# LikeLy-Journey/SegmenTron

Hardware: AMD Instinct MI355X
Metric: images/sec fwd+bwd DeepLabv3+_xception65 @1025x2049 (higher is better)
Workload: dtype bf16; 1 GPU; DeepLabv3+_xception65 train step (fwd + CE loss + bwd + SGD) @1025x2049, batch 2/GPU (BASELINE.json configs[2]); global_batch=2, bn=BN, parallelism=dp1, full_size=True

## Files before the change

### include/segmentron_hip.h

```cpp
#ifndef SEGMENTRON_HIP_H
#define SEGMENTRON_HIP_H
#ifdef __cplusplus
extern "C" {
#endif

const char* seg_last_error(void);
int seg_version(void);

int seg_fast_div_host(const int* s, long n, int d, int* q);
int seg_fast_div_exact(long s, long d);
int seg_fast_div_max_quot(long* out);

int seg_conv_gemm_fwd(int dtype, const void* x, long ldx, int N, int Hi, int Wi, int C,
                      const void* w, int O, int KH, int KW, int stride, int pad, int dil,
                      int pro_mode, const float* pro_scale, const float* pro_shift,
                      const float* bias, void* y, long ldy, int Ho, int Wo, int out_H, int out_W,
                      int out_s, float* stat_partial, const void* ep_x, long ldep,
                      const float* ep_c0, const float* ep_c1, int tconv, void* stream);
int seg_conv_gemm_tiles_m(int N, int Ho, int Wo);

int seg_conv_gemm_wgrad(int dtype, const void* x, long ldx, int N, int Hi, int Wi, int C,
                        const void* dy, long lddy, int Ho, int Wo, int O, int KH, int KW,
                        int stride, int pad, int dil, int pro_mode, const float* pro_scale,
                        const float* pro_shift, float* partial, int splits, void* stream);
int seg_conv_gemm_stat_rows(int dtype, int N, int Ho, int Wo, int C, int O, int KH, int KW,
                            int stride, int pad, int dil, int tconv, int has_bias, int pro_mode);
int seg_conv_gemm_wgrad_splits(int dtype, int N, int Ho, int Wo, int C, int O, int KH, int KW,
                               int stride, int pad, int dil, int pro_mode);

int seg_dwconv3x3(int dtype, int mode, const void* x, long ldx, int N, int Hi, int Wi, int C,
                  const float* w9c, int w_layout, int stride, int dil, int pro_mode,
                  const float* pro_scale, const float* pro_shift, void* y, long ldy, int Ho, int Wo,
                  float* stat_partial, int grid_y, void* stream);
int seg_dwconv_grid_y(int dtype, int C, int N, int Ho, int Wo, int stride, int dil, int kind);
int seg_dwconv3x3_wgrad_finalize(const float* partial, int R, int C, float* dw_c9, void* stream);
int seg_dwconv3x3_wgrad(int dtype, const void* x, long ldx, int N, int Hi, int Wi, int C,
                        const void* dy, long lddy, int Ho, int Wo, int stride, int dil,
                        int pro_mode, const float* pro_scale, const float* pro_shift,
                        float* partial, int grid_y, void* stream);

int seg_dwconv3x3_bwd_fused(int dtype, const void* dy, long lddy, const void* x, long ldx, int N,
                            int H, int W, int C, const float* w9c, int w_layout, int dil,
                            int pro_mode, const float* pro_scale, const float* pro_shift, void* g,
                            long ldg, float* partial_w, float* partial_bn, int grid_y,
                            void* stream);
int seg_dwconv3x3_bwd_fused_add_ok(int dil);
int seg_dwconv3x3_bwd_fused_add(int dtype, const void* dy, long lddy, const void* x, long ldx, int N,
                                int H, int W, int C, const float* w9c, int w_layout, int pro_mode,
                                const float* pro_scale, const float* pro_shift, const void* res,
                                long ldr, void* g, long ldg, float* partial_w, float* partial_bn,
                                int grid_y, void* stream);
int seg_dwconv3x3_bwd_fused_sum_ok(int dtype, int C, int dil);
int seg_dwconv3x3_bwd_fused_sum(int dtype, const void* dy, long lddy, const void* x, long ldx, int N,
                                int H, int W, int C, const float* w9c, int w_layout, int pro_mode,
                                const float* pro_scale, const float* pro_shift, const void* res,
                                long ldr, void* g, long ldg, float* partial_w, float* partial_bn,
                                int grid_y, void* stream);

int seg_colsum(const float* in, long R, int L, double* out_d, float* out_f, double* ws,
               void* stream);
int seg_colsum_count(const float* in, long R, int L, double* out_d, double count, double* ws,
                     void* stream);
int seg_bn_finalize(const double* sums, double count, const double* count_dev,
                    const float* gamma, const float* beta, float eps, float momentum, float* running_mean, float* running_var,
                    float* mean, float* invstd, float* scale, float* shift, int C,
                    const float* mean_offset, void* stream);
int seg_bn_finalize_p(const float* partial, long R, double count, const float* gamma,
                      const float* beta, float eps, float momentum, float* running_mean,
                      float* running_var, float* mean, float* invstd, float* scale, float* shift,
                      int C, const float* mean_offset, double* ws, void* stream);
int seg_bn_finalize_small(int dtype, const void* y, long ldy, long M, int C, const float* gamma,
                          const float* beta, float eps, float momentum, float* running_mean,
                          float* running_var, float* mean, float* invstd, float* scale,
                          float* shift, const float* mean_offset, void* stream);
int seg_bn_moments_small(int dtype, const void* y, long ldy, long M, int C, double* moments,
                         void* stream);
int seg_bn_finalize_small_sync(void* p2p, int dtype, const void* y, long ldy, long M, int C,
                               const float* gamma, const float* beta, float eps, float momentum,
                               float* running_mean, float* running_var, float* mean, float* invstd,
                               float* scale, float* shift, const float* mean_offset,
                               double* count_out, void* stream);
int seg_sum_n(int dtype, int n, const void* const* xs, const long* lds, void* y, long ldy, long M,
              int C, void* stream);
int seg_bn_eval_affine(const float* gamma, const float* beta, const float* rm, const float* rv,
                       float eps, float* scale, float* shift, int C, void* stream);
int seg_bn_eval_affine_multi(int n, const float* const* gamma, const float* const* beta,
                             const float* const* rm, const float* const* rv, const float* eps,
                             float* const* out, const int* C, void* stream);
int seg_bn_apply(int dtype, const void* x, long ldx, int mode_x, const float* sx, const float* tx,
                 const void* r, long ldr, int mode_r, const float* sr, const float* tr,
// ... 219 lines not shown
```

### segmentron_amd/csrc/dwconv_slide.hip

```cpp
#include <type_traits>
#include "common.h"
#include "dwconv.h"

namespace seg {

constexpr int SL_THREADS = 256, SL_CQ = 16, SL_WL = 16;
constexpr int SL_DEPTH_F = 2, SL_OCC_F = 4, SL_DEPTH_B = 2;
#define SL_SCHED_BARRIER() __builtin_amdgcn_sched_barrier(0)

struct DwSlideArgs {
  const void* x;
  const void* dy;
  const void* res;
  void* y;
  const float* w;
  int w_layout;
  const float* sc; const float* sh;
  float* partial;
  float* partial_bn;
  long ldx, lddy, ldy, ldr;
  int N, H, W, C, pro_mode, rs, nstrips, nwblk, ncblk;
};

struct SlBlock { int n, strip, wblk, cblk, prow; };
__device__ __forceinline__ SlBlock sl_block(const DwSlideArgs& a) {
  const int nblk = a.ncblk * a.nwblk * a.nstrips * a.N;
  int L = xcd_remap(blockIdx.x, nblk);
  SlBlock b;
  b.cblk = L % a.ncblk;
  L /= a.ncblk;
  b.prow = L;
  b.wblk = L % a.nwblk;
  L /= a.nwblk;
  b.strip = L % a.nstrips;
  b.n = L / a.nstrips;
  return b;
}

typedef float f32x2 __attribute__((ext_vector_type(2)));
typedef short s16x2 __attribute__((ext_vector_type(2)));
struct Q4 { f32x2 lo, hi; };
__device__ __forceinline__ Q4 q4_zero() { Q4 q; q.lo = q.hi = (f32x2){0.f, 0.f}; return q; }
__device__ __forceinline__ void q4_fma(Q4& acc, const Q4& a, const Q4& b) {
  acc.lo = __builtin_elementwise_fma(a.lo, b.lo, acc.lo);
  acc.hi = __builtin_elementwise_fma(a.hi, b.hi, acc.hi);
}
template <typename T> struct SlIO;
template <> struct SlIO<bf16_t> {
  typedef uint2 raw_t;
  static constexpr int BYTES = 8;
  __device__ static __forceinline__ Q4 unpack(const raw_t& r) {
    Q4 q;
    q.lo = (f32x2){__uint_as_float(r.x << 16), __uint_as_float(r.x & 0xFFFF0000u)};
    q.hi = (f32x2){__uint_as_float(r.y << 16), __uint_as_float(r.y & 0xFFFF0000u)};
// ... 60 lines not shown
      const float4 v = *reinterpret_cast<const float4*>(a.w + (long)tap * a.C + c);
      wt[k].lo = (f32x2){v.x, v.y};
      wt[k].hi = (f32x2){v.z, v.w};
    }
  }
}

template <int MODE, bool RELU_DONE>
__device__ __forceinline__ void sl_act(Q4& q, const Q4& sc, const Q4& sh) {
  const f32x2 z = {0.f, 0.f}, six = {6.f, 6.f};
  if (MODE & PRO_AFFINE) {
    q.lo = __builtin_elementwise_fma(q.lo, sc.lo, sh.lo);
    q.hi = __builtin_elementwise_fma(q.hi, sc.hi, sh.hi);
  }
  if ((MODE & PRO_RELU) && !RELU_DONE) {
    q.lo = __builtin_elementwise_max(q.lo, z);
    q.hi = __builtin_elementwise_max(q.hi, z);
  }
  if (MODE & PRO_CLAMP6) {
    q.lo = __builtin_elementwise_min(q.lo, six);
    q.hi = __builtin_elementwise_min(q.hi, six);
  }
}

struct SlThread {
  int c, w, r0, r1, rlast;
  bool live, lm, rm;
  unsigned off_m, off_0, off_p;
  bool edge, first, last;
  unsigned off_e;
  int bp_up, bp_dn;
};
template <int ESIZE>
__device__ __forceinline__ SlThread sl_thread(const DwSlideArgs& a, const SlBlock& b, long ld) {
  const int tid = threadIdx.x, cq = tid & (SL_CQ - 1), wl = tid >> 4;
  SlThread t;
  const int cfull = (b.cblk * SL_CQ + cq) * 4, wfull = b.wblk * SL_WL + wl;
  t.c = min(cfull, a.C - 4);
  t.w = min(wfull, a.W - 1);
  t.live = wfull < a.W && cfull < a.C;
  t.lm = t.w >= 1;
  t.rm = t.w + 1 < a.W;
  t.r0 = b.strip * a.rs;
  t.r1 = min(a.H, t.r0 + a.rs);
  t.rlast = min(t.r1, a.H - 1);
  t.off_m = (unsigned)((max(t.w - 1, 0) * ld + t.c) * ESIZE);
  t.off_0 = (unsigned)((t.w * ld + t.c) * ESIZE);
  t.off_p = (unsigned)((min(t.w + 1, a.W - 1) * ld + t.c) * ESIZE);
  const int lane = tid & 63, col = lane >> 4;
  t.first = col == 0;
  t.last = col == 3;
  t.edge = t.first || t.last;
  t.off_e = t.first ? t.off_m : (t.last ? t.off_p : 0xFFFFFFFFu);
  t.bp_up = ((lane - 16) & 63) * 4;
  t.bp_dn = ((lane + 16) & 63) * 4;
  return t;
}

typedef unsigned int sl_u32x2 __attribute__((ext_vector_type(2)));
typedef unsigned int sl_u32x4 __attribute__((ext_vector_type(4)));
template <typename R> __device__ __forceinline__ R sl_ld_edge(const unsigned char* row, unsigned nbytes, unsigned off);
template <> __device__ __forceinline__ uint2 sl_ld_edge<uint2>(const unsigned char* row, unsigned nbytes, unsigned off) {
  const __amdgpu_buffer_rsrc_t r = __builtin_amdgcn_make_buffer_rsrc((void*)row, 0, (int)nbytes, 0x00020000);
  const sl_u32x2 v = __builtin_amdgcn_raw_buffer_load_b64(r, (int)off, 0, 0);
  return make_uint2(v.x, v.y);
}
template <> __device__ __forceinline__ uint4 sl_ld_edge<uint4>(const unsigned char* row, unsigned nbytes, unsigned off) {
  const __amdgpu_buffer_rsrc_t r = __builtin_amdgcn_make_buffer_rsrc((void*)row, 0, (int)nbytes, 0x00020000);
  const sl_u32x4 v = __builtin_amdgcn_raw_buffer_load_b128(r, (int)off, 0, 0);
  return make_uint4(v.x, v.y, v.z, v.w);
}
template <typename R> __device__ __forceinline__ void sl_st_row(unsigned char* row, unsigned nbytes, unsigned off, const R& v);
template <> __device__ __forceinline__ void sl_st_row<uint2>(unsigned char* row, unsigned nbytes, unsigned off, const uint2& v) {
  const __amdgpu_buffer_rsrc_t r = __builtin_amdgcn_make_buffer_rsrc((void*)row, 0, (int)nbytes, 0x00020000);
  const sl_u32x2 d = {v.x, v.y};
  __builtin_amdgcn_raw_buffer_store_b64(d, r, (int)off, 0, 0);
}
template <> __device__ __forceinline__ void sl_st_row<uint4>(unsigned char* row, unsigned nbytes, unsigned off, const uint4& v) {
  const __amdgpu_buffer_rsrc_t r = __builtin_amdgcn_make_buffer_rsrc((void*)row, 0, (int)nbytes, 0x00020000);
  const sl_u32x4 d = {v.x, v.y, v.z, v.w};
  __builtin_amdgcn_raw_buffer_store_b128(d, r, (int)off, 0, 0);
// ... 296 lines not shown
#pragma unroll
  for (int k = 0; k < 9; ++k) {
    const int kw = k % 3;
    const bool keep = t.live && (kw != 2 || t.lm) && (kw != 0 || t.rm);
    v[k * 4] = keep ? accw[k].lo.x : 0.f; v[k * 4 + 1] = keep ? accw[k].lo.y : 0.f;
    v[k * 4 + 2] = keep ? accw[k].hi.x : 0.f; v[k * 4 + 3] = keep ? accw[k].hi.y : 0.f;
  }
  v[36] = s1.lo.x; v[37] = s1.lo.y; v[38] = s1.hi.x; v[39] = s1.hi.y;
  v[40] = s2.lo.x; v[41] = s2.lo.y; v[42] = s2.hi.x; v[43] = s2.hi.y;
#pragma unroll
  for (int i = 36; i < 44; ++i) v[i] = t.live ? v[i] : 0.f;
#pragma unroll
  for (int i = 0; i < 44; ++i) {
    v[i] += __shfl_xor(v[i], 16, 64);
    v[i] += __shfl_xor(v[i], 32, 64);
  }
  __shared__ float red[4][SL_CQ][44];
  if ((tid & 63) < SL_CQ) {
#pragma unroll
    for (int i = 0; i < 44; ++i) red[tid >> 6][cq][i] = v[i];
  }
  __syncthreads();
  for (int e = tid; e < SL_CQ * 44; e += SL_THREADS) {
    const int q = e / 44, k = e - q * 44;
    const float tot = red[0][q][k] + red[1][q][k] + red[2][q][k] + red[3][q][k];
    const int ch = (b.cblk * SL_CQ + q) * 4 + (k & 3), r = k >> 2;
    if (ch < a.C) {
      if (r < 9) a.partial[((long)b.prow * 9 + r) * a.C + ch] = tot;
      else if (a.partial_bn != nullptr) a.partial_bn[((long)b.prow * 2 + (r - 9)) * a.C + ch] = tot;
    }
  }
}

static void slide_geom(DwSlideArgs& a, int N, int H, int W, int C) {
  a.ncblk = (C / 4 + SL_CQ - 1) / SL_CQ;
  a.nwblk = (W + SL_WL - 1) / SL_WL;
  long ns = (H + 21) / 43;
  const long per_strip = (long)N * a.nwblk * a.ncblk;
  const long want = (400 + per_strip - 1) / per_strip;
  if (ns < want) ns = want;
  if (ns > H / 8) ns = H / 8;
  const long cap = 1024 / ((long)N * a.nwblk);
  if (ns > cap) ns = cap;
  if (ns < 1) ns = 1;
  a.rs = (int)((H + ns - 1) / ns);
  a.nstrips = (H + a.rs - 1) / a.rs;
}

int dw_slide_rows(int C, int N, int H, int W) {
  DwSlideArgs a;
  slide_geom(a, N, H, W, C);
  return N * a.nstrips * a.nwblk;
}

static bool slide_exchange(const DwSlideArgs& a, int esize) {
  return (long)a.N * a.H * a.W * a.C * esize >= (30L << 20);
}
template <typename T>
static void slide_launch_fwd(const DwSlideArgs& a, dim3 grid, hipStream_t st) {
  const bool xc = slide_exchange(a, (int)sizeof(T));
  switch (a.pro_mode) {
#define SL_CASE(M)                                                                                  \
  case M:                                                                                           \
    if (xc) hipLaunchKernelGGL((dwconv_slide_fwd_kernel<T, M, true>), grid, dim3(SL_THREADS), 0, st, a);  \
    else hipLaunchKernelGGL((dwconv_slide_fwd_kernel<T, M, false>), grid, dim3(SL_THREADS), 0, st, a);    \
    break;
    SL_CASE(0) SL_CASE(1) SL_CASE(2) SL_CASE(3) SL_CASE(5) SL_CASE(7)
#undef SL_CASE
    default: break;
  }
}
template <typename T, int RES>
static void slide_launch_bwd(const DwSlideArgs& a, dim3 grid, hipStream_t st) {
  const bool xc = slide_exchange(a, (int)sizeof(T));
  switch (a.pro_mode) {
#define SL_CASE(M)                                                                                       \
  case M:                                                                                                \
    if (xc) hipLaunchKernelGGL((dwconv_slide_bwd_kernel<T, M, RES, true>), grid, dim3(SL_THREADS), 0, st, a);  \
    else hipLaunchKernelGGL((dwconv_slide_bwd_kernel<T, M, RES, false>), grid, dim3(SL_THREADS), 0, st, a);    \
    break;
    SL_CASE(0) SL_CASE(1) SL_CASE(2) SL_CASE(3) SL_CASE(5) SL_CASE(7)
#undef SL_CASE
    default: break;
  }
}
static bool slide_mode_ok(int m) { return m == 0 || m == 1 || m == 2 || m == 3 || m == 5 || m == 7; }

int launch_dw_slide_fwd(int dtype, const void* x, long ldx, int N, int H, int W, int C,
                        const float* w, int w_layout, int pro_mode, const float* sc,
                        const float* sh, void* y, long ldy, float* stat_partial, int rows,
                        hipStream_t st) {
  DwSlideArgs a;
  a.x = x; a.dy = nullptr; a.res = nullptr; a.y = y; a.w = w; a.w_layout = w_layout;
  a.sc = sc; a.sh = sh; a.partial = stat_partial; a.partial_bn = nullptr;
  a.ldx = ldx; a.lddy = 0; a.ldy = ldy; a.ldr = 0;
  a.N = N; a.H = H; a.W = W; a.C = C; a.pro_mode = pro_mode;
  slide_geom(a, N, H, W, C);
  SEG_REQUIRE(slide_mode_ok(pro_mode), "dwconv (slide): unsupported prologue mode %d", pro_mode);
  SEG_REQUIRE(C % 4 == 0 && ldx % 4 == 0 && ldy % 4 == 0,
              "dwconv (slide): C/ldx/ldy must be multiples of 4");
  SEG_REQUIRE(stat_partial == nullptr || rows == N * a.nstrips * a.nwblk,
              "dwconv (slide): %d partial rows, the launch writes %d (seg_dwconv_grid_y)", rows,
              N * a.nstrips * a.nwblk);
  const dim3 grid((unsigned)((long)a.ncblk * a.nwblk * a.nstrips * N));
  if (dtype == DT_BF16) slide_launch_fwd<bf16_t>(a, grid, st);
  else slide_launch_fwd<float>(a, grid, st);
  return check_launch("dwconv3x3 (slide)");
}

int launch_dw_slide_bwd(int dtype, const void* dy, long lddy, const void* x, long ldx, int N, int H,
                        int W, int C, const float* w, int w_layout, int pro_mode, const float* sc,
                        const float* sh, void* g, long ldg, float* partial_w, float* partial_bn,
                        int rows, hipStream_t st, const void* res, long ldr, int res_mode) {
  DwSlideArgs a;
  a.x = x; a.dy = dy; a.res = res; a.y = g; a.w = w; a.w_layout = w_layout & 1;
  a.sc = sc; a.sh = sh; a.partial = partial_w; a.partial_bn = partial_bn;
  a.ldx = ldx; a.lddy = lddy; a.ldy = ldg; a.ldr = ldr;
  a.N = N; a.H = H; a.W = W; a.C = C; a.pro_mode = pro_mode;
  slide_geom(a, N, H, W, C);
  SEG_REQUIRE(slide_mode_ok(pro_mode), "dwconv bwd (slide): unsupported prologue mode %d", pro_mode);
  SEG_REQUIRE(C % 4 == 0 && ldx % 4 == 0 && lddy % 4 == 0 && ldg % 4 == 0 &&
                  (res == nullptr || ldr % 4 == 0),
              "dwconv bwd (slide): C/ldx/lddy/ldg/ldr must be multiples of 4");
  SEG_REQUIRE(rows == N * a.nstrips * a.nwblk,
              "dwconv bwd (slide): %d partial rows, the launch writes %d (seg_dwconv_grid_y)", rows,
              N * a.nstrips * a.nwblk);
  const dim3 grid((unsigned)((long)a.ncblk * a.nwblk * a.nstrips * N));
  const int rm = !res ? SL_RES_NONE : res_mode;
  SEG_REQUIRE(rm >= SL_RES_NONE && rm <= SL_RES_SUM, "dwconv bwd (slide): residual mode %d", rm);
  if (dtype == DT_BF16) {
    if (rm == SL_RES_SUM) slide_launch_bwd<bf16_t, SL_RES_SUM>(a, grid, st);
    else if (rm == SL_RES_POST) slide_launch_bwd<bf16_t, SL_RES_POST>(a, grid, st);
    else slide_launch_bwd<bf16_t, SL_RES_NONE>(a, grid, st);
  } else {
    if (rm == SL_RES_SUM) slide_launch_bwd<float, SL_RES_SUM>(a, grid, st);
    else if (rm == SL_RES_POST) slide_launch_bwd<float, SL_RES_POST>(a, grid, st);
    else slide_launch_bwd<float, SL_RES_NONE>(a, grid, st);
  }
  return check_launch("dwconv3x3_bwd_fused (slide)");
}

}
```

### segmentron_amd/functional.py

```python
import contextlib
import dataclasses
import os
import weakref

import torch
import torch.distributed as dist
import torch.nn as nn

from . import hip_ops as K
from . import parallel
from .hip_ops import PRO_AFFINE, PRO_NONE, PRO_RELU


class BNState:
    __slots__ = ("gamma", "beta", "mean", "invstd", "scale", "shift", "count", "training", "group")

    def __init__(self, gamma, beta, mean, invstd, scale, shift, count, training, group=None):
        self.gamma, self.beta = gamma, beta
        self.mean, self.invstd, self.scale, self.shift = mean, invstd, scale, shift
        self.count, self.training, self.group = count, training, group


RELU, RELU6 = 1, 5

# ... 336 lines not shown
    if KH == 1 and KW == 1 and opad == O:
        out = torch.empty((Cw, O), dtype=dtype, device=w.device)
        out.copy_(w.detach().reshape(O, Cw).t())
        return out
    p = w.detach().flip(2, 3).permute(1, 2, 3, 0)
    if opad != O:
        p = torch.nn.functional.pad(p, (0, opad - O))
    return p.reshape(Cw, KH * KW * opad).to(dtype).contiguous()


def pack_conv_weight_tconv(w, opad, dtype):
    O, Cw, KH, KW = w.shape
    p = w.detach().permute(1, 2, 3, 0)
    if opad != O:
        p = torch.nn.functional.pad(p, (0, opad - O))
    return p.reshape(Cw, KH * KW * opad).to(dtype).contiguous()


def pack_dw_weight(w, flipped=False):
    C = w.shape[0]
    t = w.detach().reshape(C, 9)
    if flipped:
        t = t.flip(1)
    out = torch.empty((9, C), dtype=torch.float32, device=w.device)
    out.copy_(t.t())
    return out


def _dw_taps(weight, stride, dil, reversed=False):
    if K.dw_tiled(stride, dil):
        return weight.detach()
    return cached_pack(weight, "dw_flip" if reversed else "dw",
                       lambda: pack_dw_weight(weight, reversed))


def _dw_bwd_is_fused(stride, dil, C, wdtype):
    return stride == 1 or (stride == 2 and dil == 1 and C % 4 == 0 and wdtype == torch.float32)


def _round_up(v, m):
    return (v + m - 1) // m * m


class ConvSpec:

    def __init__(self, act, stride=1, pad=0, dil=1, out=None, want_stats=True):
        self.bn_in, self.relu = act.bn, act.relu
        self.pro = act.pro
        self.stride, self.pad, self.dil = stride, pad, dil
        self.out, self.want_stats = out, want_stats
        self.partial = None
        self.drop_bias = False
        self.fork = None
        self.park = None


class _ConvFn(torch.autograd.Function):

    @staticmethod
    def forward(ctx, x, in_gamma, in_beta, weight, bias, spec):
        O, Cw, KH, KW = weight.shape
        cx, dt = x.shape[-1], x.dtype
        if KH == 1 and KW == 1 and cx == Cw and weight.dtype == torch.float32:
            wp = packed_pointwise(weight, False, dt)
        else:
            wp = cached_pack(weight, ("fwd", cx, dt), lambda: pack_conv_weight(weight, cx, dt))
# ... 125 lines not shown
        if box is not None and isinstance(bn.count, torch.Tensor):
            dgamma, dbeta, c0, c1 = K.fold_bwd_finalize_sync(
                box, dsdt, bn.count, bn.mean, bn.invstd, bn.gamma, bn.scale,
                parallel.grad_scale(bn.group))
        else:
            if bn.group is not None:
                dsdt = K.colsum(dsdt, f64=False)
                parallel.allreduce_backward_sums(dsdt, bn.group)
            dgamma, dbeta, c0, c1 = K.fold_bwd_finalize(
                dsdt, bn.count, bn.mean, bn.invstd, bn.gamma, bn.scale,
                parallel.grad_scale(bn.group) if bn.group is not None else 1.0)
        dx = None
        if ctx.needs_input_grad[0]:
            if s.stride == 1:
                dx, _ = K.conv_gemm(dy, ctx.wpt, C, 1, 1, 1, 0, 1,
                                    ep=(x, c0, c1) if bn.training else None)
            else:
                g, _ = K.conv_gemm(dy, ctx.wpt, C, 1, 1, 1, 0, 1,
                                   scatter=(x.shape[1], x.shape[2], s.stride))
                if bn.training:
                    ones = _ones(C, x.device)
                    dx = K.bn_bwd_apply(g, x, (PRO_AFFINE, ones, ones), c0, c1, out=g)
                else:
                    dx = g
            if s.park is not None and s.park.can_park(GradFork.RAW, dx, x):
                s.park.g, dx = dx, None
        return dx, dgamma, dbeta, dW.view_as(weight), None


class _DwFn(torch.autograd.Function):

    @staticmethod
    def forward(ctx, x, in_gamma, in_beta, weight, spec):
        y, spec.partial = K.dwconv(x, _dw_taps(weight, spec.stride, spec.dil), spec.stride,
                                   spec.dil, spec.pro, spec.out, spec.want_stats)
        spec.out = None
        ctx.spec = spec
        ctx.save_for_backward(x, weight)
        return y

    @staticmethod
    def backward(ctx, dy):
        x, weight = ctx.saved_tensors
        s = ctx.spec
        C = weight.shape[0]
        if K.nhwc(dy)[4] % K.vec_of(dy.dtype) != 0:
            dy = dy.contiguous()
        dx = dgamma = dbeta = None
        bn = s.bn_in
        f = s.fork
        if f is not None:
            f.closed = True
        tiled = K.dw_tiled(s.stride, s.dil)
        fused = _dw_bwd_is_fused(s.stride, s.dil, C, weight.dtype)
        fused_s2 = fused and s.stride == 2
        if ctx.needs_input_grad[0] and fused:
            raw = bn is not None and (fused_s2 or tiled) and \
                (bn.group is None or (parallel.mailbox(bn.group) is not None
                                      and isinstance(bn.count, torch.Tensor)))
            if fused_s2:
                g, dW, pb = K.dwconv_bwd_fused_s2(x, dy, weight.detach().contiguous(), s.pro,
                                                  want_bn=bn is not None, raw_dw=raw)
            else:
                res, as_sum = None, False
                if f is not None and f.g is not None and f.kind in (GradFork.POST, GradFork.SUM):
                    as_sum = f.kind == GradFork.SUM
                    if bn is None and (K.dwconv_bwd_fused_sum_ok(x.dtype, C, s.dil) if as_sum
                                       else K.dwconv_bwd_fused_add_ok(s.dil)):
                        res = s.fork.take()
                        if res.dtype != x.dtype or tuple(res.shape) != tuple(x.shape):
                            s.fork.g, res = res, None
                g, dW, pb = K.dwconv_bwd_fused(x, dy, _dw_taps(weight, 1, s.dil), s.dil, s.pro,
                                               want_bn=bn is not None, torch_layout=tiled,
                                               raw_dw=raw, res=res, res_sum=as_sum)
                if not tiled:
                    dW = K.dw_torch_layout(dW)
            if bn is None:
                dx = g
            else:
                dgamma, dbeta, c0, c1, dWsum = _bn_bwd_finish(pb, bn, dW if raw else None)
                if raw:
                    dW = dWsum
                if not bn.training:
                    c0 = c1 = None
                add = add_pro = None
                if f is not None and f.g is not None and f.kind in (GradFork.RAW, GradFork.PRE) \
                        and f.g.dtype == g.dtype and tuple(f.g.shape) == tuple(g.shape):
                    add_pro = f.coef if f.kind == GradFork.PRE else None
                    add = f.take()
                dx = K.bn_bwd_apply(g, x, (PRO_AFFINE, bn.scale, bn.shift), c0, c1, out=g, add=add,
                                    add_pro=add_pro)
        else:
            dW = K.dwconv_wgrad(x, dy, s.stride, s.dil, s.pro, torch_layout=tiled)
            if not tiled:
                dW = K.dw_torch_layout(dW)
            if ctx.needs_input_grad[0]:
                w = _dw_taps(weight, s.stride, s.dil, reversed=s.stride == 1)
                g = K.dwconv_dgrad(dy, w, s.stride, s.dil, (x.shape[1], x.shape[2]))
                dx, dgamma, dbeta = bn_input_backward(g, x, bn, s.relu, inplace=True)
        if f is not None and f.g is not None and dx is not None:
            if f.kind == GradFork.PRE:
                raise RuntimeError("a gradient parked for the depthwise backward's BatchNorm pass "
                                   "was not taken (stride %d, dilation %d, C %d)"
                                   % (s.stride, s.dil, C))
            dx = dx + f.take()
        return dx, dgamma, dbeta, dW, None

# ... 881 lines not shown
```

### segmentron_amd/hip_ops.py

```python
import torch

from ._lib import LIB

PRO_NONE, PRO_RELU, PRO_AFFINE, PRO_AFFINE_RELU = 0, 1, 2, 3
_DT = {torch.float32: 0, torch.bfloat16: 1}


def vec_of(dtype):
    return 8 if dtype == torch.bfloat16 else 4


_raw_stream = getattr(torch._C, "_cuda_getCurrentRawStream", None)


def _stream():
    if _raw_stream is not None:
        return _raw_stream(torch.cuda.current_device())
    return torch.cuda.current_stream().cuda_stream


def _p(t):
    return 0 if t is None else t.data_ptr()


# ... 249 lines not shown
def dwconv_bwd_fused_add_ok(dil):
    return bool(LIB.query("seg_dwconv3x3_bwd_fused_add_ok", int(dil)))


def dwconv_bwd_fused_sum_ok(dtype, C, dil):
    return bool(LIB.query("seg_dwconv3x3_bwd_fused_sum_ok", _DT[dtype], int(C), int(dil)))


def dwconv_bwd_fused(x, dy, w, dil, pro=None, want_bn=False, torch_layout=False, raw_dw=False,
                     res=None, out=None, res_sum=False):
    N, H, W, C, ldx = nhwc(x)
    lddy = nhwc(dy)[4]
    mode, ps, pt = _pro(pro)
    g, ldg = _dw_grad_out(out, N, H, W, C, x)
    w, layout = _dw_weight_arg(w, C, 1, dil)
    gy = _dw_grid_y("seg_dwconv_grid_y", _DT[x.dtype], C, N, H, W, 1, dil, 1)
    pw = torch.empty((gy, 9 * C), dtype=torch.float32, device=x.device)
    pb = torch.empty((gy, 2 * C), dtype=torch.float32, device=x.device) if want_bn else None
    if res is not None:
        assert dil == 1 and tuple(res.shape) == (N, H, W, C) and res.dtype == x.dtype
        LIB.call("seg_dwconv3x3_bwd_fused_sum" if res_sum else "seg_dwconv3x3_bwd_fused_add",
                 _DT[x.dtype], _p(dy), lddy, _p(x), ldx, N, H, W, C, _p(w), layout, mode, _p(ps),
                 _p(pt), _p(res), nhwc(res)[4], _p(g), ldg, _p(pw), _p(pb), gy, _stream())
    else:
        LIB.call("seg_dwconv3x3_bwd_fused", _DT[x.dtype], _p(dy), lddy, _p(x), ldx, N, H, W, C,
                 _p(w), layout, dil, mode, _p(ps), _p(pt), _p(g), ldg, _p(pw), _p(pb), gy, _stream())
    if raw_dw:
        return g, pw, pb
    if torch_layout:
        return g, dw_wgrad_finalize(pw, C), pb
    return g, colsum(pw, f64=False).view(9, C), pb


def dwconv_bwd_fused_s2(x, dy, w, pro=None, want_bn=False, raw_dw=False, out=None):
    N, H, W, C, ldx = nhwc(x)
    Nd, Ho, Wo, Cd, lddy = nhwc(dy)
    assert (Nd, Ho, Wo, Cd) == (N, (H + 1) // 2, (W + 1) // 2, C) and tuple(w.shape) == (C, 1, 3, 3)
    mode, ps, pt = _pro(pro)
    g, ldg = _dw_grad_out(out, N, H, W, C, x)
    gy = _dw_grid_y("seg_dwconv3x3_s2_grid_y", C, N, H, W)
    pw = torch.empty((gy, 9 * C), dtype=torch.float32, device=x.device)
    pb = torch.empty((gy, 2 * C), dtype=torch.float32, device=x.device) if want_bn else None
    LIB.call("seg_dwconv3x3_s2_bwd_fused", _DT[x.dtype], _p(dy), lddy, _p(x), ldx, N, H, W, C,
             _p(w), mode, _p(ps), _p(pt), _p(g), ldg, _p(pw), _p(pb), gy, _stream())
    return g, (pw if raw_dw else dw_wgrad_finalize(pw, C)), pb


def dwconv_wgrad(x, dy, stride, dil, pro=None, torch_layout=False):
    N, Hi, Wi, C, ldx = nhwc(x)
    _, Ho, Wo, _, lddy = nhwc(dy)
    mode, ps, pt = _pro(pro)
    gy = _dw_grid_y("seg_dwconv_grid_y", _DT[x.dtype], C, N, Ho, Wo, stride, dil, 2)
    partial = torch.empty((gy, 9 * C), dtype=torch.float32, device=x.device)
    LIB.call("seg_dwconv3x3_wgrad", _DT[x.dtype], _p(x), ldx, N, Hi, Wi, C, _p(dy), lddy, Ho, Wo,
             stride, dil, mode, _p(ps), _p(pt), _p(partial), gy, _stream())
    if torch_layout:
        return dw_wgrad_finalize(partial, C)
    return colsum(partial, f64=False).view(9, C)


def bn_finalize(sums, count, gamma, beta, eps, momentum, running_mean, running_var,
                mean_offset=None):
    C = sums.numel() // 2
    dev = sums.device
    out = torch.empty((4, C), dtype=torch.float32, device=dev)
    LIB.call("seg_bn_finalize", _p(sums), *_count(count), _p(gamma), _p(beta), float(eps),
# ... 827 lines not shown
```

Measured before the change: 90.10 images/sec.

## Add sliding-window depthwise 3x3 kernels for dilation-2 convolutions

Adds forward and backward HIP kernels that run the register sliding-window depthwise 3x3 scheme on dilated convolutions. Rows are split into dilation-phase chains so each chain walks with stride dil, and chains and strips are grouped per block. The Python dispatch sends stride-1, dilation-2 depthwise convs (fwd and fused bwd with BN stats) to these kernels instead of the generic dilated path. This is meant to reuse rows in registers and pipeline loads as the dil=1 path already does, at the cost of extra geometry logic and a new partial-row layout for weight-grad reductions.

```diff
diff --git a/include/segmentron_hip.h b/include/segmentron_hip.h
--- a/include/segmentron_hip.h
+++ b/include/segmentron_hip.h
@@ -56,6 +56,17 @@
                                 const float* pro_scale, const float* pro_shift, const void* res,
                                 long ldr, void* g, long ldg, float* partial_w, float* partial_bn,
                                 int grid_y, void* stream);
+
+int seg_dwconv3x3_slide_dil_rows(int dtype, int C, int N, int H, int W, int dil);
+int seg_dwconv3x3_slide_dil(int dtype, const void* x, long ldx, int N, int H, int W, int C,
+                            const float* w9c, int w_layout, int dil, int pro_mode,
+                            const float* pro_scale, const float* pro_shift, void* y, long ldy,
+                            float* stat_partial, int rows, void* stream);
+int seg_dwconv3x3_slide_dil_bwd(int dtype, const void* dy, long lddy, const void* x, long ldx, int N,
+                                int H, int W, int C, const float* w9c, int w_layout, int dil,
+                                int pro_mode, const float* pro_scale, const float* pro_shift,
+                                void* g, long ldg, float* partial_w, float* partial_bn, int rows,
+                                void* stream);
 
 int seg_colsum(const float* in, long R, int L, double* out_d, float* out_f, double* ws,
                void* stream);
diff --git a/segmentron_amd/csrc/dwconv_slide.hip b/segmentron_amd/csrc/dwconv_slide.hip
--- a/segmentron_amd/csrc/dwconv_slide.hip
+++ b/segmentron_amd/csrc/dwconv_slide.hip
@@ -20,6 +20,7 @@
   float* partial_bn;
   long ldx, lddy, ldy, ldr;
   int N, H, W, C, pro_mode, rs, nstrips, nwblk, ncblk;
+  int dil, cpb, spc;
 };
 
 struct SlBlock { int n, strip, wblk, cblk, prow; };
@@ -146,21 +147,22 @@
   int bp_up, bp_dn;
 };
 template <int ESIZE>
-__device__ __forceinline__ SlThread sl_thread(const DwSlideArgs& a, const SlBlock& b, long ld) {
+__device__ __forceinline__ SlThread sl_thread(const DwSlideArgs& a, const SlBlock& b, long ld,
+                                              int d = 1) {
   const int tid = threadIdx.x, cq = tid & (SL_CQ - 1), wl = tid >> 4;
   SlThread t;
   const int cfull = (b.cblk * SL_CQ + cq) * 4, wfull = b.wblk * SL_WL + wl;
   t.c = min(cfull, a.C - 4);
   t.w = min(wfull, a.W - 1);
   t.live = wfull < a.W && cfull < a.C;
-  t.lm = t.w >= 1;
-  t.rm = t.w + 1 < a.W;
+  t.lm = t.w >= d;
+  t.rm = t.w + d < a.W;
   t.r0 = b.strip * a.rs;
   t.r1 = min(a.H, t.r0 + a.rs);
   t.rlast = min(t.r1, a.H - 1);
-  t.off_m = (unsigned)((max(t.w - 1, 0) * ld + t.c) * ESIZE);
+  t.off_m = (unsigned)((max(t.w - d, 0) * ld + t.c) * ESIZE);
   t.off_0 = (unsigned)((t.w * ld + t.c) * ESIZE);
-  t.off_p = (unsigned)((min(t.w + 1, a.W - 1) * ld + t.c) * ESIZE);
+  t.off_p = (unsigned)((min(t.w + d, a.W - 1) * ld + t.c) * ESIZE);
   const int lane = tid & 63, col = lane >> 4;
   t.first = col == 0;
   t.last = col == 3;
@@ -523,6 +525,323 @@
   }
 }
 
+struct SlChains { int first, end, strip; };
+__device__ __forceinline__ SlChains sl_chains(const DwSlideArgs& a, const SlBlock& b) {
+  SlChains c;
+  const int group = b.strip / a.spc;
+  c.strip = b.strip - group * a.spc;
+  c.first = group * a.cpb;
+  c.end = min(min(a.dil, a.H), c.first + a.cpb);
+  return c;
+}
+struct SlWalk { int Hv, r0, r1, rlast; };
+__device__ __forceinline__ SlWalk sl_walk(const DwSlideArgs& a, const SlChains& c, int ph) {
+  SlWalk k;
+  k.Hv = (a.H - ph + a.dil - 1) / a.dil;
+  k.r0 = c.strip * a.rs;
+  k.r1 = min(k.Hv, k.r0 + a.rs);
+  k.rlast = min(k.r1, k.Hv - 1);
+  return k;
+}
+
+constexpr int SL_OCC_DIL_F = 3;
+template <typename T, int MODE, bool ROUND>
+__global__ __launch_bounds__(SL_THREADS, SL_OCC_DIL_F) void dwconv_slide_dil_fwd_kernel(const DwSlideArgs a) {
+  using IO = SlIO<T>;
+  using raw_t = typename IO::raw_t;
+  constexpr int ES = sizeof(T);
+  constexpr bool RAWRELU = IO::RAW_RELU && MODE == PRO_RELU;
+  static_assert(!ROUND || (std::is_same<T, bf16_t>::value && (MODE & PRO_AFFINE)), "ROUND: bf16 + affine");
+  const int tid = threadIdx.x, cq = tid & (SL_CQ - 1);
+  const SlBlock b = sl_block(a);
+  const SlThread t = sl_thread<ES>(a, b, a.ldx, a.dil);
+  const SlChains ch = sl_chains(a, b);
+
+  Q4 wt[9], sc, sh;
+  sc = sh = q4_zero();
+  const unsigned char* __restrict__ Xb = reinterpret_cast<const unsigned char*>(a.x) +
+                                         (long)b.n * a.H * a.W * a.ldx * ES;
+  unsigned char* __restrict__ Yb = reinterpret_cast<unsigned char*>(a.y) +
+                                   (long)b.n * a.H * a.W * a.ldy * ES;
+  const long xrow = (long)a.W * a.ldx * ES, yrow = (long)a.W * a.ldy * ES;
+  const long xpitch = xrow * a.dil, ypitch = yrow * a.dil;
+  const unsigned yoff = t.live ? (unsigned)((t.w * a.ldy + t.c) * ES) : 0xFFFFFFFFu;
+  const unsigned char* __restrict__ Xc = Xb;
+  unsigned char* __restrict__ Yc = Yb;
+  SlWalk k = {0, 0, 0, 0};
+
+  auto issue = [&](int r, raw_t (&raw)[3]) {
+    const unsigned char* __restrict__ row = Xc + (long)min(max(r, 0), k.rlast) * xpitch;
+    raw[0] = sl_ld<raw_t>(row, t.off_0);
+    raw[1] = sl_ld<raw_t>(row, t.off_m);
+    raw[2] = sl_ld<raw_t>(row, t.off_p);
+  };
+  auto commit = [&](int r, const raw_t (&raw)[3], Q4 (&row)[3], auto check) {
+    constexpr bool CHECK = decltype(check)::value;
+    const bool rv = !CHECK || (r >= 0 && r < k.Hv);
+    const raw_t r3[3] = {raw[1], raw[0], raw[2]};
+#pragma unroll
+    for (int j = 0; j < 3; ++j) {
+      row[j] = IO::unpack(RAWRELU ? IO::relu_raw(r3[j]) : r3[j]);
+      sl_act<MODE, RAWRELU>(row[j], sc, sh);
+      if (ROUND) row[j] = IO::unpack(IO::pack(row[j]));
+      if (CHECK && !rv) row[j] = q4_zero();
+    }
+  };
+  Q4 ssum = q4_zero(), ssq = q4_zero();
+  auto compute = [&](int ro, const Q4 (&ra)[3], const Q4 (&rb)[3], const Q4 (&rc)[3]) {
+    Q4 acc = q4_zero();
+#pragma unroll
+    for (int kw = 0; kw < 3; ++kw) q4_fma(acc, ra[kw], wt[kw]);
+#pragma unroll
+    for (int kw = 0; kw < 3; ++kw) q4_fma(acc, rb[kw], wt[3 + kw]);
+#pragma unroll
+    for (int kw = 0; kw < 3; ++kw) q4_fma(acc, rc[kw], wt[6 + kw]);
+    sl_st_row<raw_t>(Yc + (long)ro * ypitch, (unsigned)yrow, yoff, IO::pack(acc));
+    ssum.lo += acc.lo; ssum.hi += acc.hi;
+    q4_fma(ssq, acc, acc);
+  };
+
+  constexpr int D = SL_DEPTH_F, U = (D % 3 == 0) ? D : 3 * D;
+  Q4 win[3][3];
+  raw_t ring[D][3];
+  bool params = false;
+  for (int ph = ch.first; ph < ch.end; ++ph) {
+    k = sl_walk(a, ch, ph);
+    if (k.r0 >= k.r1) continue;
+    const int r0 = k.r0, r1 = k.r1;
+    Xc = Xb + ph * xrow;
+    Yc = Yb + ph * yrow;
+#pragma unroll
+    for (int j = 0; j < D; ++j) issue(r0 - 1 + j, ring[j]);
+    if (!params) {
+      params = true;
+      sl_load_taps(a, t.c, wt);
+      if (MODE & PRO_AFFINE) {
+        const float4 s4 = *reinterpret_cast<const float4*>(a.sc + t.c);
+        const float4 t4 = *reinterpret_cast<const float4*>(a.sh + t.c);
+        sc.lo = (f32x2){s4.x, s4.y}; sc.hi = (f32x2){s4.z, s4.w};
+        sh.lo = (f32x2){t4.x, t4.y}; sh.hi = (f32x2){t4.z, t4.w};
+      }
+#pragma unroll
+      for (int kh = 0; kh < 3; ++kh) {
+        if (!t.lm) wt[kh * 3] = q4_zero();
+        if (!t.rm) wt[kh * 3 + 2] = q4_zero();
+      }
+    }
+    commit(r0 - 1, ring[0], win[0], std::true_type{});
+    issue(r0 - 1 + D, ring[0]);
+    commit(r0, ring[1 % D], win[1], std::false_type{});
+    issue(r0 + D, ring[1 % D]);
+    int ro = r0;
+    for (; ro + U < r1; ro += U) {
+#pragma unroll
+      for (int j = 0; j < U; ++j) {
+        commit(ro + j + 1, ring[(j + 2) % D], win[(j + 2) % 3], std::false_type{});
+        issue(ro + j + 1 + D, ring[(j + 2) % D]);
+        SL_SCHED_BARRIER();
+        compute(ro + j, win[j % 3], win[(j + 1) % 3], win[(j + 2) % 3]);
+        SL_SCHED_BARRIER();
+      }
+    }
+#pragma unroll
+    for (int j = 0; j < U; ++j) {
+      if (ro + j < r1) {
+        commit(ro + j + 1, ring[(j + 2) % D], win[(j + 2) % 3], std::true_type{});
+        issue(ro + j + 1 + D, ring[(j + 2) % D]);
+        compute(ro + j, win[j % 3], win[(j + 1) % 3], win[(j + 2) % 3]);
+      }
+    }
+  }
+
+  if (a.partial != nullptr) {
+    __shared__ float red[4][SL_CQ][8];
+    float v[8] = {ssum.lo.x, ssum.lo.y, ssum.hi.x, ssum.hi.y, ssq.lo.x, ssq.lo.y, ssq.hi.x, ssq.hi.y};
+#pragma unroll
+    for (int i = 0; i < 8; ++i) {
+      v[i] = t.live ? v[i] : 0.f;
+      v[i] += __shfl_xor(v[i], 16, 64);
+      v[i] += __shfl_xor(v[i], 32, 64);
+    }
+    if ((tid & 63) < SL_CQ) {
+#pragma unroll
+      for (int i = 0; i < 8; ++i) red[tid >> 6][cq][i] = v[i];
+    }
+    __syncthreads();
+    if (tid < SL_CQ * 8) {
+      const int q = tid >> 3, i = tid & 7;
+      const float tot = red[0][q][i] + red[1][q][i] + red[2][q][i] + red[3][q][i];
+      const int c = (b.cblk * SL_CQ + q) * 4 + (i & 3);
+      if (c < a.C) a.partial[((long)b.prow * 2 + (i >> 2)) * a.C + c] = tot;
+    }
+  }
+}
+
+template <typename T, int MODE>
+__global__ __launch_bounds__(SL_THREADS, 2) void dwconv_slide_dil_bwd_kernel(const DwSlideArgs a) {
+  using IO = SlIO<T>;
+  using raw_t = typename IO::raw_t;
+  constexpr int ES = sizeof(T);
+  const int tid = threadIdx.x, cq = tid & (SL_CQ - 1);
+  const SlBlock b = sl_block(a);
+  const SlThread t = sl_thread<ES>(a, b, a.lddy, a.dil);
+  const SlChains ch = sl_chains(a, b);
+
+  Q4 wt[9], sc, sh;
+  sc = sh = q4_zero();
+  const long img = (long)b.n * a.H * a.W;
+  const unsigned char* __restrict__ Db = reinterpret_cast<const unsigned char*>(a.dy) + img * a.lddy * ES;
+  const unsigned char* __restrict__ Xb = reinterpret_cast<const unsigned char*>(a.x) + img * a.ldx * ES;
+  unsigned char* __restrict__ Gb = reinterpret_cast<unsigned char*>(a.y) + img * a.ldy * ES;
+  const long drow = (long)a.W * a.lddy * ES, xrow = (long)a.W * a.ldx * ES;
+  const long grow = (long)a.W * a.ldy * ES;
+  const long dpitch = drow * a.dil, xpitch = xrow * a.dil, gpitch = grow * a.dil;
+  const unsigned xoff = (unsigned)((t.w * a.ldx + t.c) * ES);
+  const unsigned goff = t.live ? (unsigned)((t.w * a.ldy + t.c) * ES) : 0xFFFFFFFFu;
+  const unsigned char* __restrict__ Dc = Db;
+  const unsigned char* __restrict__ Xc = Xb;
+  unsigned char* __restrict__ Gc = Gb;
+  SlWalk k = {0, 0, 0, 0};
+
+  auto issue = [&](int r, raw_t (&raw)[3]) {
+    const unsigned char* __restrict__ row = Dc + (long)min(max(r, 0), k.rlast) * dpitch;
+    raw[0] = sl_ld<raw_t>(row, t.off_0);
+    raw[1] = sl_ld<raw_t>(row, t.off_m);
+    raw[2] = sl_ld<raw_t>(row, t.off_p);
+  };
+  auto issue_x = [&](int r, raw_t& xr) {
+    xr = sl_ld<raw_t>(Xc + (long)min(r, k.r1 - 1) * xpitch, xoff);
+  };
+  auto commit = [&](int r, const raw_t (&raw)[3], Q4 (&row)[3], auto check) {
+    constexpr bool CHECK = decltype(check)::value;
+    const bool rv = !CHECK || (r >= 0 && r < k.Hv);
+    const raw_t r3[3] = {raw[1], raw[0], raw[2]};
+#pragma unroll
+    for (int j = 0; j < 3; ++j) {
+      row[j] = IO::unpack(r3[j]);
+      if (CHECK && !rv) row[j] = q4_zero();
+    }
+  };
+  Q4 accw[9], s1 = q4_zero(), s2 = q4_zero();
+#pragma unroll
+  for (int j = 0; j < 9; ++j) accw[j] = q4_zero();
+
+  auto compute = [&](int ro, const raw_t& xraw, const Q4 (&ra)[3], const Q4 (&rb)[3],
+                     const Q4 (&rcw)[3]) {
+    const Q4 xr = IO::unpack(xraw);
+    Q4 xa = xr;
+    sl_act<MODE, false>(xa, sc, sh);
+    Q4 g = q4_zero();
+#pragma unroll
+    for (int bq = 0; bq < 3; ++bq) { q4_fma(g, ra[bq], wt[8 - bq]); q4_fma(accw[8 - bq], ra[bq], xa); }
+#pragma unroll
+    for (int bq = 0; bq < 3; ++bq) { q4_fma(g, rb[bq], wt[5 - bq]); q4_fma(accw[5 - bq], rb[bq], xa); }
+#pragma unroll
+    for (int bq = 0; bq < 3; ++bq) { q4_fma(g, rcw[bq], wt[2 - bq]); q4_fma(accw[2 - bq], rcw[bq], xa); }
+    if (MODE & PRO_RELU) {
+      auto on = [&](float v) { return v > 0.f && (!(MODE & PRO_CLAMP6) || v < 6.f); };
+      g.lo.x = on(xa.lo.x) ? g.lo.x : 0.f; g.lo.y = on(xa.lo.y) ? g.lo.y : 0.f;
+      g.hi.x = on(xa.hi.x) ? g.hi.x : 0.f; g.hi.y = on(xa.hi.y) ? g.hi.y : 0.f;
+    }
+    sl_st_row<raw_t>(Gc + (long)ro * gpitch, (unsigned)grow, goff, IO::pack(g));
+    s1.lo += g.lo; s1.hi += g.hi;
+    q4_fma(s2, g, xr);
+  };
+
+  constexpr int D = SL_DEPTH_B, U = (D % 3 == 0) ? D : 3 * D;
+  Q4 win[3][3];
+  raw_t ring[D][3], xring[D];
+  bool params = false;
+  for (int ph = ch.first; ph < ch.end; ++ph) {
+    k = sl_walk(a, ch, ph);
+    if (k.r0 >= k.r1) continue;
+    const int r0 = k.r0, r1 = k.r1;
+    Dc = Db + ph * drow;
+    Xc = Xb + ph * xrow;
+    Gc = Gb + ph * grow;
+#pragma unroll
+    for (int j = 0; j < D; ++j) {
+      issue(r0 - 1 + j, ring[j]);
+      issue_x(r0 + j, xring[j]);
+    }
+    if (!params) {
+      params = true;
+      sl_load_taps(a, t.c, wt);
+      if (MODE & PRO_AFFINE) {
+        const float4 s4 = *reinterpret_cast<const float4*>(a.sc + t.c);
+        const float4 t4 = *reinterpret_cast<const float4*>(a.sh + t.c);
+        sc.lo = (f32x2){s4.x, s4.y}; sc.hi = (f32x2){s4.z, s4.w};
+        sh.lo = (f32x2){t4.x, t4.y}; sh.hi = (f32x2){t4.z, t4.w};
+      }
+#pragma unroll
+      for (int kh = 0; kh < 3; ++kh) {
+        if (!t.lm) wt[kh * 3 + 2] = q4_zero();
+        if (!t.rm) wt[kh * 3] = q4_zero();
+      }
+    }
+    commit(r0 - 1, ring[0], win[0], std::true_type{});
+    issue(r0 - 1 + D, ring[0]);
+    commit(r0, ring[1 % D], win[1], std::false_type{});
+    issue(r0 + D, ring[1 % D]);
+    int ro = r0;
+    for (; ro + U < r1; ro += U) {
+#pragma unroll
+      for (int j = 0; j < U; ++j) {
+        commit(ro + j + 1, ring[(j + 2) % D], win[(j + 2) % 3], std::false_type{});
+        issue(ro + j + 1 + D, ring[(j + 2) % D]);
+        const raw_t xraw = xring[j % D];
+        issue_x(ro + j + D, xring[j % D]);
+        SL_SCHED_BARRIER();
+        compute(ro + j, xraw, win[j % 3], win[(j + 1) % 3], win[(j + 2) % 3]);
+        SL_SCHED_BARRIER();
+      }
+    }
+#pragma unroll
+    for (int j = 0; j < U; ++j) {
+      if (ro + j < r1) {
+        commit(ro + j + 1, ring[(j + 2) % D], win[(j + 2) % 3], std::true_type{});
+        issue(ro + j + 1 + D, ring[(j + 2) % D]);
+        const raw_t xraw = xring[j % D];
+        issue_x(ro + j + D, xring[j % D]);
+        compute(ro + j, xraw, win[j % 3], win[(j + 1) % 3], win[(j + 2) % 3]);
+      }
+    }
+  }
+
+  float v[44];
+#pragma unroll
+  for (int j = 0; j < 9; ++j) {
+    const int kw = j % 3;
+    const bool keep = t.live && (kw != 2 || t.lm) && (kw != 0 || t.rm);
+    v[j * 4] = keep ? accw[j].lo.x : 0.f; v[j * 4 + 1] = keep ? accw[j].lo.y : 0.f;
+    v[j * 4 + 2] = keep ? accw[j].hi.x : 0.f; v[j * 4 + 3] = keep ? accw[j].hi.y : 0.f;
+  }
+  v[36] = s1.lo.x; v[37] = s1.lo.y; v[38] = s1.hi.x; v[39] = s1.hi.y;
+  v[40] = s2.lo.x; v[41] = s2.lo.y; v[42] = s2.hi.x; v[43] = s2.hi.y;
+#pragma unroll
+  for (int i = 36; i < 44; ++i) v[i] = t.live ? v[i] : 0.f;
+#pragma unroll
+  for (int i = 0; i < 44; ++i) {
+    v[i] += __shfl_xor(v[i], 16, 64);
+    v[i] += __shfl_xor(v[i], 32, 64);
+  }
+  __shared__ float red[4][SL_CQ][44];
+  if ((tid & 63) < SL_CQ) {
+#pragma unroll
+    for (int i = 0; i < 44; ++i) red[tid >> 6][cq][i] = v[i];
+  }
+  __syncthreads();
+  for (int e = tid; e < SL_CQ * 44; e += SL_THREADS) {
+    const int q = e / 44, i = e - q * 44;
+    const float tot = red[0][q][i] + red[1][q][i] + red[2][q][i] + red[3][q][i];
+    const int c = (b.cblk * SL_CQ + q) * 4 + (i & 3), r = i >> 2;
+    if (c < a.C) {
+      if (r < 9) a.partial[((long)b.prow * 9 + r) * a.C + c] = tot;
+      else if (a.partial_bn != nullptr) a.partial_bn[((long)b.prow * 2 + (r - 9)) * a.C + c] = tot;
+    }
+  }
+}
+
 static void slide_geom(DwSlideArgs& a, int N, int H, int W, int C) {
   a.ncblk = (C / 4 + SL_CQ - 1) / SL_CQ;
   a.nwblk = (W + SL_WL - 1) / SL_WL;
@@ -586,6 +905,7 @@
   a.sc = sc; a.sh = sh; a.partial = stat_partial; a.partial_bn = nullptr;
   a.ldx = ldx; a.lddy = 0; a.ldy = ldy; a.ldr = 0;
   a.N = N; a.H = H; a.W = W; a.C = C; a.pro_mode = pro_mode;
+  a.dil = 1; a.cpb = a.spc = 1;
   slide_geom(a, N, H, W, C);
   SEG_REQUIRE(slide_mode_ok(pro_mode), "dwconv (slide): unsupported prologue mode %d", pro_mode);
   SEG_REQUIRE(C % 4 == 0 && ldx % 4 == 0 && ldy % 4 == 0,
@@ -608,6 +928,7 @@
   a.sc = sc; a.sh = sh; a.partial = partial_w; a.partial_bn = partial_bn;
   a.ldx = ldx; a.lddy = lddy; a.ldy = ldg; a.ldr = ldr;
   a.N = N; a.H = H; a.W = W; a.C = C; a.pro_mode = pro_mode;
+  a.dil = 1; a.cpb = a.spc = 1;
   slide_geom(a, N, H, W, C);
   SEG_REQUIRE(slide_mode_ok(pro_mode), "dwconv bwd (slide): unsupported prologue mode %d", pro_mode);
   SEG_REQUIRE(C % 4 == 0 && ldx % 4 == 0 && lddy % 4 == 0 && ldg % 4 == 0 &&
@@ -631,4 +952,133 @@
   return check_launch("dwconv3x3_bwd_fused (slide)");
 }
 
-}
+constexpr int SL_DIL_ROWS = 16;
+static bool slide_dil_geom(DwSlideArgs& a, int N, int H, int W, int C, int dil) {
+  a.ncblk = (C / 4 + SL_CQ - 1) / SL_CQ;
+  a.nwblk = (W + SL_WL - 1) / SL_WL;
+  a.dil = dil;
+  const int nch = dil < H ? dil : H, hv = (H + dil - 1) / dil;
+  const long per_unit = (long)N * a.nwblk;
+  if (per_unit > 1024) return false;
+  a.cpb = 1;
+  a.spc = 1;
+  if (2 * hv > 3 * SL_DIL_ROWS) a.spc = (hv + SL_DIL_ROWS / 2) / SL_DIL_ROWS;
+  else if (hv < SL_DIL_ROWS) a.cpb = SL_DIL_ROWS / hv;
+  while (a.spc > 1 && per_unit * nch * a.spc > 1024) --a.spc;
+  if (a.cpb > nch) a.cpb = nch;
+  while (per_unit * ((nch + a.cpb - 1) / a.cpb) * a.spc > 1024) ++a.cpb;
+  a.rs = (hv + a.spc - 1) / a.spc;
+  a.nstrips = ((nch + a.cpb - 1) / a.cpb) * a.spc;
+  return true;
+}
+
+static int slide_dil_rows(int dtype, int C, int N, int H, int W, int dil) {
+  if ((dtype != DT_F32 && dtype != DT_BF16) || C < 4 || C % 4 != 0 || N < 1 || H < 1 || W < 1 ||
+      dil < 2)
+    return -1;
+  DwSlideArgs a;
+  if (!slide_dil_geom(a, N, H, W, C, dil)) return -1;
+  return N * a.nstrips * a.nwblk;
+}
+
+template <typename T>
+static void slide_dil_launch_fwd(const DwSlideArgs& a, dim3 grid, hipStream_t st) {
+  switch (a.pro_mode) {
+#define SL_CASE(M)                                                                                   \
+  case M:                                                                                            \
+    if constexpr (std::is_same<T, bf16_t>::value && ((M) & PRO_AFFINE) != 0) {                        \
+      if (a.dil == 2) {                                                                              \
+        hipLaunchKernelGGL((dwconv_slide_dil_fwd_kernel<T, M, true>), grid, dim3(SL_THREADS), 0, st, a); \
+        break;                                                                                       \
+      }                                                                                              \
+    }                                                                                                \
+    hipLaunchKernelGGL((dwconv_slide_dil_fwd_kernel<T, M, false>), grid, dim3(SL_THREADS), 0, st, a);  \
+    break;
+    SL_CASE(0) SL_CASE(1) SL_CASE(2) SL_CASE(3) SL_CASE(5) SL_CASE(7)
+#undef SL_CASE
+    default: break;
+  }
+}
+template <typename T>
+static void slide_dil_launch_bwd(const DwSlideArgs& a, dim3 grid, hipStream_t st) {
+  switch (a.pro_mode) {
+#define SL_CASE(M)                                                                             \
+  case M:                                                                                      \
+    hipLaunchKernelGGL((dwconv_slide_dil_bwd_kernel<T, M>), grid, dim3(SL_THREADS), 0, st, a); \
+    break;
+    SL_CASE(0) SL_CASE(1) SL_CASE(2) SL_CASE(3) SL_CASE(5) SL_CASE(7)
+#undef SL_CASE
+    default: break;
+  }
+}
+
+}
+
+extern "C" int seg_dwconv3x3_slide_dil_rows(int dtype, int C, int N, int H, int W, int dil) {
+  return seg::slide_dil_rows(dtype, C, N, H, W, dil);
+}
+
+extern "C" int seg_dwconv3x3_slide_dil(int dtype, const void* x, long ldx, int N, int H, int W,
+                                       int C, const float* w9c, int w_layout, int dil,
+                                       int pro_mode, const float* pro_scale,
+                                       const float* pro_shift, void* y, long ldy,
+                                       float* stat_partial, int rows, void* stream) {
+  using namespace seg;
+  const int want = slide_dil_rows(dtype, C, N, H, W, dil);
+  SEG_REQUIRE(want >= 1, "dwconv3x3_slide_dil: no such launch (dtype %d, C %d, %d x %d x %d, "
+              "dilation %d)", dtype, C, N, H, W, dil);
+  SEG_REQUIRE(slide_mode_ok(pro_mode), "dwconv3x3_slide_dil: unsupported prologue mode %d", pro_mode);
+  SEG_REQUIRE(((pro_mode & PRO_AFFINE) == 0) || (pro_scale && pro_shift),
+              "dwconv3x3_slide_dil: affine prologue without scale/shift");
+  SEG_REQUIRE(ldx % 4 == 0 && ldy % 4 == 0 && ldx >= C && ldy >= C,
+              "dwconv3x3_slide_dil: ldx/ldy must be multiples of 4, at least C");
+  SEG_REQUIRE(w_layout == 0 || w_layout == 1, "dwconv3x3_slide_dil: tap layout %d", w_layout);
+  SEG_REQUIRE(rows == want, "dwconv3x3_slide_dil: %d partial rows, the launch writes %d "
+              "(seg_dwconv3x3_slide_dil_rows)", rows, want);
+  SEG_REQUIRE((long)W * (ldx > ldy ? ldx : ldy) * 4 < (1L << 32),
+              "dwconv3x3_slide_dil: an image row exceeds 32-bit byte offsets");
+  DwSlideArgs a;
+  a.x = x; a.dy = nullptr; a.res = nullptr; a.y = y; a.w = w9c; a.w_layout = w_layout;
+  a.sc = pro_scale; a.sh = pro_shift; a.partial = stat_partial; a.partial_bn = nullptr;
+  a.ldx = ldx; a.lddy = 0; a.ldy = ldy; a.ldr = 0;
+  a.N = N; a.H = H; a.W = W; a.C = C; a.pro_mode = pro_mode;
+  slide_dil_geom(a, N, H, W, C, dil);
+  const dim3 grid((unsigned)((long)a.ncblk * a.nwblk * a.nstrips * N));
+  if (dtype == DT_BF16) slide_dil_launch_fwd<bf16_t>(a, grid, (hipStream_t)stream);
+  else slide_dil_launch_fwd<float>(a, grid, (hipStream_t)stream);
+  return check_launch("dwconv3x3_slide_dil");
+}
+
+extern "C" int seg_dwconv3x3_slide_dil_bwd(int dtype, const void* dy, long lddy, const void* x,
+                                           long ldx, int N, int H, int W, int C, const float* w9c,
+                                           int w_layout, int dil, int pro_mode,
+                                           const float* pro_scale, const float* pro_shift, void* g,
+                                           long ldg, float* partial_w, float* partial_bn, int rows,
+                                           void* stream) {
+  using namespace seg;
+  const int want = slide_dil_rows(dtype, C, N, H, W, dil);
+  SEG_REQUIRE(want >= 1, "dwconv3x3_slide_dil_bwd: no such launch (dtype %d, C %d, %d x %d x %d, "
+              "dilation %d)", dtype, C, N, H, W, dil);
+  SEG_REQUIRE(slide_mode_ok(pro_mode), "dwconv3x3_slide_dil_bwd: unsupported prologue mode %d",
+              pro_mode);
+  SEG_REQUIRE(((pro_mode & PRO_AFFINE) == 0) || (pro_scale && pro_shift),
+              "dwconv3x3_slide_dil_bwd: affine prologue without scale/shift");
+  SEG_REQUIRE(ldx % 4 == 0 && lddy % 4 == 0 && ldg % 4 == 0 && ldx >= C && lddy >= C && ldg >= C,
+              "dwconv3x3_slide_dil_bwd: ldx/lddy/ldg must be multiples of 4, at least C");
+  SEG_REQUIRE(w_layout == 0 || w_layout == 1, "dwconv3x3_slide_dil_bwd: tap layout %d", w_layout);
+  SEG_REQUIRE(partial_w != nullptr && rows == want, "dwconv3x3_slide_dil_bwd: %d partial rows, the "
+              "launch writes %d (seg_dwconv3x3_slide_dil_rows)", rows, want);
+  const long ldmax = ldx > lddy ? (ldx > ldg ? ldx : ldg) : (lddy > ldg ? lddy : ldg);
+  SEG_REQUIRE((long)W * ldmax * 4 < (1L << 32),
+              "dwconv3x3_slide_dil_bwd: an image row exceeds 32-bit byte offsets");
+  DwSlideArgs a;
+  a.x = x; a.dy = dy; a.res = nullptr; a.y = g; a.w = w9c; a.w_layout = w_layout;
+  a.sc = pro_scale; a.sh = pro_shift; a.partial = partial_w; a.partial_bn = partial_bn;
+  a.ldx = ldx; a.lddy = lddy; a.ldy = ldg; a.ldr = 0;
+  a.N = N; a.H = H; a.W = W; a.C = C; a.pro_mode = pro_mode;
+  slide_dil_geom(a, N, H, W, C, dil);
+  const dim3 grid((unsigned)((long)a.ncblk * a.nwblk * a.nstrips * N));
+  if (dtype == DT_BF16) slide_dil_launch_bwd<bf16_t>(a, grid, (hipStream_t)stream);
+  else slide_dil_launch_bwd<float>(a, grid, (hipStream_t)stream);
+  return check_launch("dwconv3x3_slide_dil_bwd");
+}
diff --git a/segmentron_amd/functional.py b/segmentron_amd/functional.py
--- a/segmentron_amd/functional.py
+++ b/segmentron_amd/functional.py
@@ -392,6 +392,18 @@
         return weight.detach()
     return cached_pack(weight, "dw_flip" if reversed else "dw",
                        lambda: pack_dw_weight(weight, reversed))
+
+
+_NO_SLIDE_DIL = os.environ.get("SEG_NO_SLIDE_DIL") == "1"
+_SLIDE_DIL_MAX = 2
+
+
+def _dw_slide_dil(stride, dil, *tensors):
+    if _NO_SLIDE_DIL or stride != 1 or dil < 2 or dil > _SLIDE_DIL_MAX:
+        return False
+    N, H, W, C, _ = K.nhwc(tensors[0])
+    return all(t is None or K.nhwc(t)[4] % 4 == 0 for t in tensors) and \
+        K.dwconv_slide_dil_rows(tensors[0].dtype, C, N, H, W, dil) >= 1
 
 
 def _dw_bwd_is_fused(stride, dil, C, wdtype):
@@ -583,8 +595,12 @@
 
     @staticmethod
     def forward(ctx, x, in_gamma, in_beta, weight, spec):
-        y, spec.partial = K.dwconv(x, _dw_taps(weight, spec.stride, spec.dil), spec.stride,
-                                   spec.dil, spec.pro, spec.out, spec.want_stats)
+        if _dw_slide_dil(spec.stride, spec.dil, x, spec.out):
+            y, spec.partial = K.dwconv_slide_dil(x, weight.detach(), spec.dil, spec.pro, spec.out,
+                                                 spec.want_stats)
+        else:
+            y, spec.partial = K.dwconv(x, _dw_taps(weight, spec.stride, spec.dil), spec.stride,
+                                       spec.dil, spec.pro, spec.out, spec.want_stats)
         spec.out = None
         ctx.spec = spec
         ctx.save_for_backward(x, weight)
@@ -602,7 +618,8 @@
         f = s.fork
         if f is not None:
             f.closed = True
-        tiled = K.dw_tiled(s.stride, s.dil)
+        slide_dil = _dw_slide_dil(s.stride, s.dil, x, dy)
+        tiled = K.dw_tiled(s.stride, s.dil) or slide_dil
         fused = _dw_bwd_is_fused(s.stride, s.dil, C, weight.dtype)
         fused_s2 = fused and s.stride == 2
         if ctx.needs_input_grad[0] and fused:
@@ -621,9 +638,14 @@
                         res = s.fork.take()
                         if res.dtype != x.dtype or tuple(res.shape) != tuple(x.shape):
                             s.fork.g, res = res, None
-                g, dW, pb = K.dwconv_bwd_fused(x, dy, _dw_taps(weight, 1, s.dil), s.dil, s.pro,
-                                               want_bn=bn is not None, torch_layout=tiled,
-                                               raw_dw=raw, res=res, res_sum=as_sum)
+                if slide_dil:
+                    g, dW, pb = K.dwconv_slide_dil_bwd(x, dy, weight.detach(), s.dil, s.pro,
+                                                       want_bn=bn is not None, torch_layout=True,
+                                                       raw_dw=raw)
+                else:
+                    g, dW, pb = K.dwconv_bwd_fused(x, dy, _dw_taps(weight, 1, s.dil), s.dil, s.pro,
+                                                   want_bn=bn is not None, torch_layout=tiled,
+                                                   raw_dw=raw, res=res, res_sum=as_sum)
                 if not tiled:
                     dW = K.dw_torch_layout(dW)
             if bn is None:
diff --git a/segmentron_amd/hip_ops.py b/segmentron_amd/hip_ops.py
--- a/segmentron_amd/hip_ops.py
+++ b/segmentron_amd/hip_ops.py
@@ -305,6 +305,50 @@
     return g, colsum(pw, f64=False).view(9, C), pb
 
 
+def dwconv_slide_dil_rows(dtype, C, N, H, W, dil):
+    return LIB.query("seg_dwconv3x3_slide_dil_rows", _DT[dtype], int(C), int(N), int(H), int(W),
+                     int(dil))
+
+
+def _dw_slide_dil_taps(w, C):
+    if w.dim() == 4 or (w.dim() == 2 and w.shape == (C, 9) and C != 9):
+        return w, 1
+    return w, 0
+
+
+def dwconv_slide_dil(x, w, dil, pro=None, out=None, want_stats=False):
+    N, H, W, C, ldx = nhwc(x)
+    mode, ps, pt = _pro(pro)
+    if out is None:
+        out = torch.empty((N, H, W, C), dtype=x.dtype, device=x.device)
+    ldy = nhwc(out)[4]
+    w, layout = _dw_slide_dil_taps(w, C)
+    rows = _dw_grid_y("seg_dwconv3x3_slide_dil_rows", _DT[x.dtype], C, N, H, W, dil)
+    partial = torch.empty((rows, 2, C), dtype=torch.float32, device=x.device) if want_stats else None
+    LIB.call("seg_dwconv3x3_slide_dil", _DT[x.dtype], _p(x), ldx, N, H, W, C, _p(w), layout, dil,
+             mode, _p(ps), _p(pt), _p(out), ldy, _p(partial), rows, _stream())
+    return out, partial
+
+
+def dwconv_slide_dil_bwd(x, dy, w, dil, pro=None, want_bn=False, torch_layout=False, raw_dw=False,
+                         out=None):
+    N, H, W, C, ldx = nhwc(x)
+    lddy = nhwc(dy)[4]
+    mode, ps, pt = _pro(pro)
+    g, ldg = _dw_grad_out(out, N, H, W, C, x)
+    w, layout = _dw_slide_dil_taps(w, C)
+    rows = _dw_grid_y("seg_dwconv3x3_slide_dil_rows", _DT[x.dtype], C, N, H, W, dil)
+    pw = torch.empty((rows, 9 * C), dtype=torch.float32, device=x.device)
+    pb = torch.empty((rows, 2 * C), dtype=torch.float32, device=x.device) if want_bn else None
+    LIB.call("seg_dwconv3x3_slide_dil_bwd", _DT[x.dtype], _p(dy), lddy, _p(x), ldx, N, H, W, C,
+             _p(w), layout, dil, mode, _p(ps), _p(pt), _p(g), ldg, _p(pw), _p(pb), rows, _stream())
+    if raw_dw:
+        return g, pw, pb
+    if torch_layout:
+        return g, dw_wgrad_finalize(pw, C), pb
+    return g, colsum(pw, f64=False).view(9, C), pb
+
+
 def dwconv_bwd_fused_s2(x, dy, w, pro=None, want_bn=False, raw_dw=False, out=None):
     N, H, W, C, ldx = nhwc(x)
     Nd, Ho, Wo, Cd, lddy = nhwc(dy)
```

Measured after the change: 90.76 images/sec (median of 6 runs). Within noise of the previous version (+0.7%).
